# OpenVQE/OpenVQE

Measured on AMD Instinct MI355X. Metric: vqe_energy_evals_per_sec, higher is better.
Workload: dtype f64; 1 GPU; H2O/STO-3G UCCSD energy evaluation (the metric's config): 14 qubits, 140 generators = 1000 Pauli rotations, JW Hamiltonian 1086 terms / 162 x-groups; batch_per_gpu=65536, parallelism=batch-replicas x1

## Files before the change

openvqe_amd/backend.py:

```python
from __future__ import annotations

import ctypes
import os

import numpy as np

from . import _lib
from .operators import pack_string, pack_terms

GATE_OPCODES = {"X": 0, "H": 1, "RX": 2, "RY": 3, "RZ": 4, "CNOT": 5}
GRAD_FERMIONIC, GRAD_QUBIT = 0, 1
_REAL_TOL = 1e-12


def _real_coeff(c, what):
    c = complex(c)
    if abs(c.imag) > _REAL_TOL * max(1.0, abs(c.real)):
        raise ValueError(f"{what}: Pauli coefficient {c} is not real (generator must be Hermitian — "
                         "multiply the anti-Hermitian cluster operator by 1j, ref:openvqe/algorithms/ucc.py:30-31)")
    return c.real


def compile_ucc_program(nbqbits, generators, n_params=None):
    K = len(generators) if n_params is None else min(len(generators), int(n_params))
# ... 550 lines not shown
        cap = max(int(getattr(self, "_ham_terms", 0)), 1)
        got = np.full(cap, -1, np.int32)
        xb = np.zeros(cap, np.uint64)
        yb = np.zeros(cap, np.uint64)
        self._ck(self._L.ovqe_measure_groups(self._h, cap, got, xb, yb, ctypes.byref(G)))
        return got[:int(getattr(self, "_ham_terms", 0))], xb[:G.value], yb[:G.value]

    def energy_sampled(self, theta, n_shots, seed=0):
        K = self._K
        theta = np.ascontiguousarray(theta, np.float64).reshape(-1)[:K]
        if theta.shape[0] != K:
            raise ValueError(f"expected {K} parameters")
        e, s = ctypes.c_double(), ctypes.c_double()
        self._ck(self._L.ovqe_energy_sampled(self._h, theta if K else None, K, int(n_shots), int(seed), ctypes.byref(e), ctypes.byref(s)))
        return e.value, s.value

    def measure_info(self):
        out = (ctypes.c_int64 * 9)()
        self._ck(self._L.ovqe_measure_info(self._h, out, 9))
        keys = ("groups", "shots", "scratch_bytes", "launches", "basis_us", "scan_us", "draw_us", "terms", "high_passes")
        return dict(zip(keys, [int(v) for v in out]))

    def program_info(self):
        out = (ctypes.c_int64 * 38)()
        self._ck(self._L.ovqe_program_info(self._h, out, 38))
        keys = ("ops", "rotations", "literal_gates", "sweeps", "tiled_sweeps", "fused_ops", "support",
                "h_tile_sweeps", "h_untiled_groups", "h_entries", "h_merged_terms", "h_pair_terms_per_tile",
                "real_stream", "sp_ops", "sp_pairs", "sp_h_entries",
                "sector_support", "sector_sweeps", "sector_pairs", "sector_h_sweeps", "sector_h_elements", "sector_bytes",
                "sector_circuit_us", "sector_expect_us", "sector_h_stream_bytes", "sector_fci_block",
                "sp_conflicts_discovery_order", "sp_conflicts", "sector_regular_slot_bits", "sector_free_bits",
                "sp_h_pieces", "sp_h_slots", "sp_h_reads_per_state",
                "sp_lds_row_reads", "sp_lds_row_writes", "sp_lds_h_reads",
                "sp_lds_row_reads_discovery_order", "sp_lds_row_writes_discovery_order")
        return dict(zip(keys, [int(v) for v in out]))

    def rotation_program(self):
        n = ctypes.c_int64()
        self._ck(self._L.ovqe_get_rotation_program(self._h, 0, None, None, None, None, None, ctypes.byref(n)))
        R = n.value
        xs, zs = np.empty(R, np.uint64), np.empty(R, np.uint64)
        cs, p0, pi = np.empty(R, np.float64), np.empty(R, np.float64), np.empty(R, np.int32)
        self._ck(self._L.ovqe_get_rotation_program(self._h, R, xs.ctypes.data, zs.ctypes.data, cs.ctypes.data, p0.ctypes.data,
                                                   pi.ctypes.data, ctypes.byref(n)))
        return xs, zs, cs, p0, pi

    def pool_gradients(self, pool_ops, mode):
        cache = getattr(self, "_pool_cache", None)
        if cache is not None and cache[0] is pool_ops and cache[1] == len(pool_ops):
            offsets, xs, zs, cs = cache[2]
        else:
            offsets = np.zeros(len(pool_ops) + 1, np.int64)
            xs, zs, cs = [], [], []
            for k, op in enumerate(pool_ops):
                px, pz, pc = pack_terms(self.nbqbits, op.terms)
                xs.append(px)
                zs.append(pz)
# ... 34 lines not shown
```

openvqe_amd/csrc/ovqe_sv.hip:

```cpp
#include "../../include/ovqe_sv.h"

#include <hip/hip_runtime.h>

#include <algorithm>
#include <type_traits>
#include <atomic>
#include <cmath>
#include <cstdio>
#include <complex>
#include <cstring>
#include <map>
#include <memory>
#include <numeric>
#include <string>
#include <thread>
#include <chrono>
#include <vector>

#include "sv_kernels.hpp"
#include "sv_small.hpp"
#include "sv_sparse.hpp"
#include "sparse_pack.hpp"
#include "sv_tile.hpp"
#include "sv_sector.hpp"
// ... 259 lines not shown
    HamDev ham_adhoc;
    std::vector<uint64_t> adhoc_x, adhoc_z;
    std::vector<double> adhoc_c;
    bool prog_set = false;
    int32_t K = 0;
    uint64_t hf = 0;
    std::vector<SmallOp> ops;
    std::vector<SmallRot> rots;
    std::vector<SmallOp> sops;
    std::vector<SmallRot> srots;
    std::vector<int32_t> sop_src;
    std::vector<uint64_t> sop_zc;
    std::vector<SmallSeg> segs;
    DevBuf d_ops, d_rots, d_segs, d_stream;
    DevBuf d_rots_seq;
    std::vector<uint16_t> idx_stream;
    int cs_capacity = 512;
    DevBuf d_theta, d_energies, d_workspace;
    bool sp_tried = false, sp_valid = false;
    int sp_m = 0, sp_nops = 0, sp_nent = 0;
    int sp_nrows4 = 0;
    int sp_nprim = 0;
    DevBuf d_sp_rows, d_sp_rows64, d_sp_prim;
    int sp_nrows8 = 0;
    int sp_mp = 0, sp_hf = 0;
    int64_t sp_conflicts_before = 0, sp_conflicts_after = 0;
    int64_t sp_cycles[5] = {0, 0, 0, 0, 0};
    int64_t sp_npairs = 0;
    DevBuf d_sp_ops, d_sp_pairs, d_sp_entries;
    int sp_pack_inst = -1, sp_h_pieces = 0, sp_h_rpt = 0, sp_h_epr = 0;
    DevBuf d_sp_hpack;
    DevBuf d_pg_off, d_pg_xs, d_pg_terms, d_pg_out, d_pg_part;
    DevBuf d_pg_runs, d_pg_tabs;
    bool pg_tables = false;
    DevBuf d_nz_cnt, d_nz_start, d_nz_idx, d_nz_val, d_nz_bitmap;
    DevBuf d_exp_groups, d_exp_terms;
    std::vector<uint64_t> prev_x, prev_z;
    std::vector<double> prev_coeff, prev_phi0;
    std::vector<int32_t> prev_pidx;
    uint64_t prev_hf = 0;
    bool prog_extends_prev = false;
    uint32_t forms_used = 0;
    uint32_t sp_forms = 0;
    int64_t fused_launch[6] = {0, 0, 0, 0, 0, 0};
    bool nz_super = false, nz_super_prev = false, state_exposed = false;
    uint64_t nz_super_count = 0;
    DevBuf d_tile_smasks, d_tile_lists, d_tile_counts;
    int opt_screen_sparse = 16;
    int64_t last_exp_support = -1;
    int64_t last_screen_sector = 0;
    int64_t last_screen_support = -1;
    std::vector<int64_t> pg_off;
    std::vector<uint64_t> pg_xs;
    std::vector<HTerm> pg_terms;
    bool pg_valid = false;
    int opt_sparse = 1;
    int opt_sparse_spw = 0;
    int opt_sparse_pack = 1;
    int opt_sparse_dbg = 0;
    int opt_clifford_phase_host = 1;
    int opt_sparse_renumber = 1;
    int opt_sparse_rows = 1;
    int opt_sparse_wg = 1;
    int opt_sparse_shared = 1;
    int opt_sparse_grad = 1;
    DevBuf d_egroups, d_eterms, d_echunks, d_eflat;
    int exp_lbits = -1, exp_real = -1, exp_ngroups = 0, exp_nchunks = 0, exp_nflat = 0;
    int exp_ham_version = -1;
    hipEvent_t ev0 = nullptr, ev1 = nullptr;
    hipStream_t stream2 = nullptr;
    hipEvent_t ev_fork = nullptr, ev_join = nullptr;
    int opt_real_state = 0;
    CompactCover cc;
    int opt_compact = 1;
    int prog_version = 0;
    SectorEngine sec;
    SectorEngine scr;
    int scr_failed_version = -1;
    bool probe_independent = false;
    int opt_sector = 1;
    int opt_sector_bits = 0;
// ... 732 lines not shown
    return create_common(n_qubits, 0, 0, device, out);
} OVQE_CATCH(nullptr)

int ovqe_create_shard(int n_local, int n_global, uint64_t shard_index, int device, ovqe_handle *out) try {
    return create_common(n_local, n_global, shard_index, device, out);
} OVQE_CATCH(nullptr)

int ovqe_create_view(int n_qubits, int device, void *dev_ptr, ovqe_handle *out) try {
    if (!dev_ptr) return fail(nullptr, OVQE_ERR_INVALID, "dev_ptr is NULL");
    return create_common(n_qubits, 0, 0, device, out, dev_ptr);
} OVQE_CATCH(nullptr)

int ovqe_destroy(ovqe_handle h) try {
    OVQE_ENTER(h);
    if (!h) return OVQE_OK;
    (void)hipSetDevice(h->device);
    (void)hipStreamSynchronize(h->stream);
    if (h->own_state && h->state) (void)hipFree(h->state);
    for (int k = 0; k < 2; ++k)
        if (h->scratch[k]) (void)hipFree(h->scratch[k]);
    std::vector<DevBuf *> bufs = {&h->d_tile_cnt, &h->d_partials, &h->d_result, &h->d_rp, &h->d_ops, &h->d_rots, &h->d_rots_seq, &h->d_segs,
                                  &h->d_stream,
                                  &h->d_theta, &h->d_energies, &h->d_workspace, &h->d_egroups, &h->d_eterms, &h->d_echunks,
                                  &h->d_eflat, &h->d_sp_ops, &h->d_sp_rows, &h->d_sp_rows64, &h->d_sp_prim, &h->d_sp_pairs, &h->d_sp_entries, &h->d_sp_hpack, &h->d_pg_off, &h->d_pg_xs, &h->d_pg_terms, &h->d_pg_runs, &h->d_pg_tabs,
                                  &h->d_pg_out, &h->d_pg_part, &h->d_nz_cnt, &h->d_nz_start, &h->d_nz_idx, &h->d_nz_val, &h->d_nz_bitmap, &h->d_exp_groups, &h->d_exp_terms, &h->d_tile_smasks, &h->d_tile_lists, &h->d_tile_counts, &h->cc.d_sup, &h->cc.d_psic, &h->cc.d_loc, &h->cc.d_cid, &h->cc.d_off, &h->cc.d_sweeps};
    for (TilePlan *tp : {&h->tp, &h->tp_adhoc, &h->tp_real, &h->tp_adjoint}) bufs.insert(bufs.end(), {&tp->d_tops, &tp->d_trots});
    for (HamDev *H : {&h->ham, &h->ham_adhoc, &h->ham_real, &h->ham_conj})
        bufs.insert(bufs.end(), {&H->d_groups, &H->d_terms, &H->d_tchunks, &H->d_tgroups, &H->d_tterms, &H->d_tflats,
                                 &H->d_titems, &H->d_rest, &H->d_achunks, &H->d_agroups, &H->d_aterms, &H->d_dzin, &H->d_doff, &H->d_dterms});
    for (DevBuf *b : bufs)
        if (b->p) (void)hipFree(b->p);
    free_sector(h->sec);
    free_sector(h->scr);
    for (CrossSum *X : h->xsums) free_cross_sum(X);
    for (PoolPlan *P : h->xpools) free_pool_plan(P);
    free_rdm(h->rdm);
    free_metric(h->metric);
    free_measure(h->measure);
    free_subspace(h->subspace);
    h->kept_blocks.flush();
    if (h->h_rp) (void)hipHostFree(h->h_rp);
    if (h->h_result) (void)hipHostFree(h->h_result);
    if (h->h_io) (void)hipHostFree(h->h_io);
    if (h->h_fin) (void)hipHostFree(h->h_fin);
    if (h->ev0) (void)hipEventDestroy(h->ev0);
    if (h->ev1) (void)hipEventDestroy(h->ev1);
    if (h->ev_fork) (void)hipEventDestroy(h->ev_fork);
// ... 22 lines not shown
    OVQE_ENTER(h);
    if (!h || !name) return OVQE_ERR_INVALID;
    const std::string k(name);
    if (k == "force_path") h->opt_force_path = (int)value;
    else if (k == "real_state") h->opt_real_state = value ? 1 : 0;
    else if (k == "small_max_qubits") h->opt_small_max = (int)value;
    else if (k == "small_batch_max_qubits") h->opt_small_batch_max = (int)value;
    else if (k == "real_mode") {
        h->opt_real_mode = (int)value;
        h->sp_tried = false;
    }
    else if (k == "sparse") {
        h->opt_sparse = (int)value;
        h->sp_tried = false;
    }
    else if (k == "sparse_grad") h->opt_sparse_grad = value ? 1 : 0;
    else if (k == "sparse_renumber") {
        h->opt_sparse_renumber = value ? 1 : 0;
        h->sp_tried = false;
    }
#ifdef OVQE_TESTING
    else if (k == "sparse_spw") h->opt_sparse_spw = (int)value;
    else if (k == "sparse_dbg") h->opt_sparse_dbg = (int)value;
    else if (k == "sparse_pack") {
        h->opt_sparse_pack = value ? 1 : 0;
        h->sp_tried = false;
    }
#endif
    else if (k == "clifford_phase_host") h->opt_clifford_phase_host = (int)value;
    else if (k == "index_streams") {
        h->opt_index_streams = (int)value;
        if (h->prog_set) return finish_program(h);
    }
    else if (k == "sector" || k == "sector_bits" || k == "sector_max_gb" || k == "sector_min_qubits" || k == "sector_h" ||
             k == "sector_h_bits" || k == "sector_dict") {
        (k == "sector" ? h->opt_sector : k == "sector_bits" ? h->opt_sector_bits : k == "sector_max_gb" ? h->opt_sector_max_gb
         : k == "sector_h" ? h->opt_sector_h : k == "sector_h_bits" ? h->opt_sector_h_bits : k == "sector_dict" ? h->opt_sector_dict
                                                                                                              : h->opt_sector_min_qubits) = (int)value;
        reset_sector(h);
    }
    else if (k == "sector_threads") h->opt_sector_threads = (value == 0 || value == 64 || value == 512 || value == 1024) ? (int)value : 256;
#ifdef OVQE_TESTING
    else if (k == "sector_h_dbg") h->opt_sector_h_dbg = (int)value;
#endif
    else if (k == "sector_adjoint") h->opt_sector_adjoint = value == 1 ? 1 : (value == 2 ? 2 : 3);
    else if (k == "sector_batch") h->opt_sector_batch = (int)value;
// ... 256 lines not shown
    const TilePlan &TP = (real_on && h->tp_real_built) ? h->tp_real : h->tp;
    int64_t v[16] = {(int64_t)h->ops.size(), (int64_t)h->rots.size(), 0, (int64_t)TP.plan.size(),
                     (int64_t)TP.tsegs.size(), (int64_t)h->sops.size(),
                     !h->sp_tried ? -1 : (h->sp_valid ? (int64_t)h->sp_m : 0),
                     (int64_t)HI.tsweeps.size(), (int64_t)HI.n_rest, HI.tile_entries, HI.tile_terms, HI.tile_work,
                     real_on ? 1 : 0, h->sp_valid ? (int64_t)h->sp_nops : 0, h->sp_valid ? (int64_t)h->sp_npairs : 0,
                     h->sp_valid ? (int64_t)h->sp_nent : 0};
    for (const SmallOp &op : h->ops) v[2] += (op.kind == OP_X || op.kind == OP_H || op.kind == OP_CNOT);
    for (int i = 0; i < count && i < 16; ++i) info[i] = v[i];
    const SectorEngine &E = h->sec;
    const int64_t sv[14] = {E.valid ? (int64_t)E.K : 0, E.valid ? (int64_t)E.segs.size() : 0, E.valid ? (int64_t)E.npairs : 0,
                           E.valid ? (int64_t)E.hs.size() : 0, E.valid ? (int64_t)E.nnz : 0, E.valid ? (int64_t)E.bytes : 0,
                           E.valid ? (int64_t)(1e3 * E.last_circuit_ms) : 0, E.valid ? (int64_t)(1e3 * E.last_expect_ms) : 0,
                           E.valid ? (int64_t)E.h_stream_bytes : 0, E.valid ? (int64_t)E.last_fci_block : 0,
                            h->sp_valid ? h->sp_conflicts_before : 0, h->sp_valid ? h->sp_conflicts_after : 0,
                            (E.valid && E.regular && h->opt_sector_regular) ? (int64_t)E.reg_m : 0,
                            (E.valid && E.regular) ? (int64_t)__builtin_popcount(E.freemask) : 0};
    for (int i = 16; i < count && i < 30; ++i) info[i] = sv[i - 16];
    const bool packed = h->sp_valid && h->sp_pack_inst >= 0;
    const int64_t pv[3] = {packed ? (int64_t)h->sp_h_pieces : 0, packed ? (int64_t)h->sp_h_rpt * h->sp_h_epr : 0,
                           packed ? (int64_t)h->sp_h_rpt * (h->sp_h_epr + 1) : 0};
    for (int i = 30; i < count && i < 33; ++i) info[i] = pv[i - 30];
    for (int i = 33; i < count && i < 38; ++i) info[i] = h->sp_valid ? h->sp_cycles[i - 33] : 0;
    return OVQE_OK;
} OVQE_CATCH(h)

int ovqe_get_rotation_program(ovqe_handle h, int64_t capacity, uint64_t *x, uint64_t *z, double *coeff, double *phi0,
                              int32_t *pidx, int64_t *count) try {
    OVQE_ENTER(h);
    if (!h || !count || capacity < 0 || (capacity > 0 && (!x || !z || !coeff || !phi0 || !pidx))) return OVQE_ERR_INVALID;
    if (!h->prog_set) return fail(h, OVQE_ERR_STATE, "no program set");
    if (h->frame_open) return fail(h, OVQE_ERR_STATE, "the program's Clifford frame is open: the rotations alone are not the circuit");
    int64_t n = 0;
    for (const SmallOp &op : h->ops) {
        if (op.kind != OP_PAIR && op.kind != OP_DIAG) return fail(h, OVQE_ERR_STATE, "the program holds literal X / H / CNOT ops");
        for (int32_t r = op.first; r < op.first + op.count; ++r, ++n) {
            if (n >= capacity) continue;
            const SmallRot &sr = h->rots[r];
            x[n] = op.x;
            z[n] = sr.z;
            coeff[n] = sr.coeff;
            phi0[n] = sr.phi0;
            pidx[n] = sr.pidx;
        }
    }
    *count = n;
// ... 24 lines not shown
```

openvqe_amd/csrc/sparse_host.inc:

```

struct SharedInstance { int nw, ept, sstride, rpt, epr, te; };
constexpr SharedInstance SHARED_13 = {4, 13, 2568, 1, 17, 3};
constexpr SharedInstance SHARED_37 = {4, 37, 4104, 4, 10, 5};
constexpr SharedInstance SHARED_INSTANCES[2] = {SHARED_13, SHARED_37};

int build_sparse_program(ovqe_handle h) {
    h->sp_tried = true;
    h->sp_valid = false;
    if (!h->opt_sparse || !h->opt_table_fusion || !h->opt_real_mode || h->n_global != 0 || h->n_local > 40) return OVQE_OK;
    if (!h->prog_set || !h->ham.set || h->K <= 0) return OVQE_OK;
    for (const SmallRot &sr : h->rots)
        if (!(sr.ny & 1)) return OVQE_OK;
    for (const SmallOp &op : h->sops)
        if (op.kind != OP_TAB || op.count > 127) return OVQE_OK;
    const int MAXM = 4096;
    std::unordered_map<uint64_t, int> id;
    std::vector<uint64_t> S;
    auto get = [&](uint64_t a) {
        auto it = id.find(a);
        if (it != id.end()) return it->second;
        const int k = (int)S.size();
        id.emplace(a, k);
        S.push_back(a);
        return k;
// ... 49 lines not shown
            if (d == 0.0) continue;
            SpEntry e;
            e.ij = (uint32_t)k | ((uint32_t)kb << 12);
            e.pad = 0;
            e.c = x ? 2.0 * d : d;
            entries.push_back(e);
            if (entries.size() > (size_t)16 << 20) return OVQE_OK;
        }
    }
    SparsePlan plan;
    {
        std::vector<PlanOp> pops;
        for (const SpOp &so : ops) pops.push_back({so.first, so.npairs});
        plan_sparse_program(m, pops, pairs, h->opt_sparse_renumber != 0, &plan);
    }
    pairs.swap(plan.pairs);
    const int mp = plan.mp, hf_slot = plan.slot[0];
    h->sp_conflicts_before = plan.conflicts_discovery;
    h->sp_conflicts_after = plan.conflicts;
    for (SpEntry &e : entries) e.ij = (uint32_t)plan.slot[e.ij & 0xfffu] | ((uint32_t)plan.slot[(e.ij >> 12) & 0xfffu] << 12);
    arrange_entries(entries);
    std::vector<uint64_t> rows;
    h->sp_nrows4 = 0;
    const int ntab_all = (int)h->srots.size();
    std::vector<SmallRot> prim;
    std::vector<int> prim_of((size_t)ntab_all, -1);
    std::vector<uint8_t> prim_neg((size_t)ntab_all, 0);
    {
        std::unordered_map<uint64_t, std::vector<int>> by_param;
        for (int e = 0; e < ntab_all; ++e) {
            const SmallRot &sr = h->srots[e];
            std::vector<int> &cand = by_param[(uint64_t)(uint32_t)sr.pidx];
            for (int p : cand)
                if (std::fabs(prim[p].coeff) == std::fabs(sr.coeff) && prim[p].phi0 == 0.0 && sr.phi0 == 0.0) {
                    prim_of[e] = p;
                    prim_neg[e] = (prim[p].coeff < 0) != (sr.coeff < 0);
                    break;
                }
            if (prim_of[e] < 0) {
                prim_of[e] = (int)prim.size();
                cand.push_back((int)prim.size());
                prim.push_back(sr);
            }
        }
    }
    const int nprim = (int)prim.size();
// ... 3 lines not shown
            return (uint64_t)((uint32_t)(mp + lane) * 8u) | ((uint64_t)((uint32_t)(mp + 32 + lane) * 8u) << 16) |
                   ((uint64_t)((uint32_t)nprim * 16u) << 32);
        };
        size_t at = 0;
        for (const SpOp &so : ops)
            for (int c0 = 0; c0 < so.npairs; c0 += 32)
                for (int lane = 0; lane < 32; ++lane) {
                    const RowLane &rl = plan.rows[at++];
                    const uint64_t slots = (uint64_t)(rl.si * 8u) | ((uint64_t)(rl.sj * 8u) << 16);
                    if (rl.pair < 0) {
                        rows.push_back(slots | ((uint64_t)((uint32_t)nprim * 16u) << 32));
                        continue;
                    }
                    const uint32_t pw = pairs[(size_t)rl.pair], ent = (uint32_t)so.tab0 + (pw >> 25);
                    const bool neg = ((pw >> 24) & 1u) != (uint32_t)prim_neg[ent];
                    rows.push_back(slots | ((uint64_t)((uint32_t)prim_of[ent] * 16u) << 32) | (neg ? (1ull << 63) : 0ull));
                }
        const int nrows = (int)(rows.size() / 32);
        const int nrows4 = (nrows + 3) & ~3;
        for (int r = nrows; r < nrows4 + 4; ++r)
            for (int lane = 0; lane < 32; ++lane) rows.push_back(pad_word(lane));
        h->sp_nrows4 = nrows4;
        h->sp_nprim = nprim;
    }
    std::vector<uint64_t> rows64;
    h->sp_nrows8 = 0;
    if (h->opt_sparse_rows && (size_t)(mp + 128) * 8 < 65536 && (size_t)(nprim + 1) * 16 < 65536) {
        auto pad_word = [&](int lane) {
            return (uint64_t)((uint32_t)(mp + lane) * 8u) | ((uint64_t)((uint32_t)(mp + 64 + lane) * 8u) << 16) |
                   ((uint64_t)((uint32_t)nprim * 16u) << 32);
        };
        size_t at = 0;
        for (const SpOp &so : ops) {
            const int nch = (so.npairs + 31) / 32;
            for (int c = 0; c < nch; c += 2) {
                const int halves = std::min(2, nch - c);
                uint32_t ent0 = (uint32_t)nprim;
                for (int l = 0; l < 32 * halves; ++l)
                    if (plan.rows[at + l].pair >= 0) {
                        ent0 = (uint32_t)prim_of[(uint32_t)so.tab0 + (pairs[(size_t)plan.rows[at + l].pair] >> 25)];
                        break;
                    }
                for (int hh = 0; hh < 2; ++hh)
                    for (int l = 0; l < 32; ++l) {
                        if (hh >= halves) {
                            rows64.push_back((pad_word(32 + l) & 0xffffffffull) | ((uint64_t)(ent0 * 16u) << 32));
// ... 34 lines not shown
            ei[e] = entries[e].ij & 0xfffu;
            ej[e] = (entries[e].ij >> 12) & 0xfffu;
            ec[e] = entries[e].c;
        }
        const size_t state_bytes = (size_t)((mp + 64 + 1) & ~1) * sizeof(double);
        for (int k = 0; k < 2 && h->sp_pack_inst < 0; ++k) {
            const SharedInstance &I = SHARED_INSTANCES[k];
            const int nt = 64 * I.nw;
            if (entries.size() > (size_t)nt * I.ept || state_bytes > (size_t)I.sstride) continue;
            OwnerPack P;
            if (!pack_owner_pieces(ei, ej, ec, mp, nt, I.rpt, I.epr, &P)) continue;
            hpack.resize(P.c.size() * sizeof(double) + (P.oj.size() + P.oi.size()) * sizeof(uint16_t));
            std::memcpy(hpack.data(), P.c.data(), P.c.size() * sizeof(double));
            std::memcpy(hpack.data() + P.c.size() * sizeof(double), P.oj.data(), P.oj.size() * sizeof(uint16_t));
            std::memcpy(hpack.data() + P.c.size() * sizeof(double) + P.oj.size() * sizeof(uint16_t), P.oi.data(), P.oi.size() * sizeof(uint16_t));
            h->sp_pack_inst = k;
            h->sp_h_pieces = P.pieces;
            h->sp_h_rpt = I.rpt;
            h->sp_h_epr = I.epr;
            const PackCycles pc = pack_cycles(P);
            h->sp_cycles[2] = pc.slot_reads + pc.owner_reads;
        }
    }
    int rc = upload(h, h->d_sp_ops, ops.data(), ops.size() * sizeof(SpOp));
    if (!rc && h->sp_pack_inst >= 0) rc = upload(h, h->d_sp_hpack, hpack.data(), hpack.size());
    if (!rc && h->sp_nrows4) rc = upload(h, h->d_sp_rows, rows.data(), rows.size() * sizeof(uint64_t));
    if (!rc && (h->sp_nrows4 || h->sp_nrows8)) rc = upload(h, h->d_sp_prim, prim.data(), prim.size() * sizeof(SmallRot));
    if (!rc && h->sp_nrows8) rc = upload(h, h->d_sp_rows64, rows64.data(), rows64.size() * sizeof(uint64_t));
    if (!rc) rc = upload(h, h->d_sp_pairs, pairs.data(), pairs.size() * sizeof(uint32_t));
    if (!rc) rc = upload(h, h->d_sp_entries, entries.data(), entries.size() * sizeof(SpEntry));
    if (rc) return rc;
    h->sp_m = m;
    h->sp_mp = mp;
    h->sp_hf = hf_slot;
    h->sp_nops = (int)ops.size();
    h->sp_nent = (int)entries.size();
    h->sp_npairs = (int64_t)pairs.size();
    h->sp_valid = true;
    return OVQE_OK;
}

template <int SPW, bool STAGE = false>
int launch_sparse(ovqe_handle h, const SparseArgs &A, int grid, size_t smem) {
    if (int rc = lds_opt_in<&k_sparse_vqe<SPW, STAGE>>(h, LDS_WG_MAX)) return rc;
    hipLaunchKernelGGL((k_sparse_vqe<SPW, STAGE>), dim3(grid), dim3(64), smem, h->stream, A, h->cur_theta,
                       (const SmallRot *)h->d_rots.p, (const SpOp *)h->d_sp_ops.p, (const uint32_t *)h->d_sp_pairs.p,
                       (const SpEntry *)h->d_sp_entries.p, h->cur_energies);
    HIPC(h, hipGetLastError());
    return OVQE_OK;
}

enum : uint32_t {
    SPF_WG = 1u << 0,
    SPF_STAGED1 = 1u << 1,
    SPF_PLAIN1 = 1u << 2,
    SPF_ROWS2 = 1u << 3,
    SPF_PLAIN2 = 1u << 4,
    SPF_PLAIN4 = 1u << 5,
    SPF_GRAD_WG = 1u << 6,
    SPF_GRAD_STAGED = 1u << 7,
    SPF_GRAD_PLAIN = 1u << 8,
    SPF_DECLINED = 1u << 9,
    SPG_PER_WAVE = 1u << 10,
    SPG_SHARED_37 = 1u << 11,
    SPG_SHARED_13 = 1u << 12,
};

constexpr int64_t SHARED_MIN_B = 2048;

template <int NW, int RPT, int EPR, int SSTRIDE, int TE, int DBG>
int launch_rows_shared_dbg(ovqe_handle h, const SparseArgs &R, size_t smem) {
    constexpr int NS = 2 * NW;
    static std::atomic<uint32_t> per_dev[64];
    constexpr auto kern = &k_sparse_vqe_rows_shared<NW, RPT, EPR, SSTRIDE, TE, DBG>;
    constexpr size_t slots = (size_t)RPT * EPR * NW * 64;
    const double *hc = (const double *)h->d_sp_hpack.p;
    const uint16_t *ho = (const uint16_t *)(hc + slots);
    if (int rc = lds_opt_in<kern>(h, LDS_WG_MAX)) return rc;
    uint32_t pd = per_dev[h->device & 63].load(std::memory_order_relaxed);
    if ((pd >> 8) != smem) {
        int n = 0;
        HIPC(h, hipOccupancyMaxActiveBlocksPerMultiprocessor(&n, kern, NW * 64, smem));
        pd = (uint32_t)smem << 8 | (uint32_t)std::min(std::max(n, 1), 32 / NW);
        per_dev[h->device & 63].store(pd, std::memory_order_relaxed);
    }
    const int per_cu = (int)(pd & 255u);
    if (h->num_cus <= 0) {
        int cus = 0;
        if (hipDeviceGetAttribute(&cus, hipDeviceAttributeMultiprocessorCount, h->device) != hipSuccess || cus <= 0) cus = 256;
        h->num_cus = cus;
    }
    const int grid = (int)std::min<int64_t>((R.B + NS - 1) / NS, (int64_t)h->num_cus * per_cu);
    hipLaunchKernelGGL(kern, dim3(grid), dim3(NW * 64), smem, h->stream, R, h->cur_theta, (const SmallRot *)h->d_sp_prim.p,
                       (const uint64_t *)h->d_sp_rows.p, h->sp_nrows4, hc, ho, h->cur_energies);
    HIPC(h, hipGetLastError());
    return OVQE_OK;
}

template <int K>
int launch_rows_shared(ovqe_handle h, const SparseArgs &R, bool *taken) {
    constexpr SharedInstance I = SHARED_INSTANCES[K];
    constexpr int NW = I.nw, RPT = I.rpt, EPR = I.epr, SSTRIDE = I.sstride, TE = I.te;
    const size_t smem = sp_rows_shared_lds<NW, SSTRIDE>(R.ntab).bytes;
    *taken = h->sp_pack_inst == K && R.nent >= 1 && R.nent <= NW * 64 * I.ept && (size_t)R.mpad * sizeof(double) <= (size_t)SSTRIDE &&
             smem <= LDS_TWO_PER_CU;
    if (!*taken) return OVQE_OK;
#ifdef OVQE_TESTING
    switch (h->opt_sparse_dbg) {
    case 1: return launch_rows_shared_dbg<NW, RPT, EPR, SSTRIDE, TE, 1>(h, R, smem);
    case 2: return launch_rows_shared_dbg<NW, RPT, EPR, SSTRIDE, TE, 2>(h, R, smem);
    case 3: return launch_rows_shared_dbg<NW, RPT, EPR, SSTRIDE, TE, 3>(h, R, smem);
    case 4: return launch_rows_shared_dbg<NW, RPT, EPR, SSTRIDE, TE, 4>(h, R, smem);
    case 5: return launch_rows_shared_dbg<NW, RPT, EPR, SSTRIDE, TE, 5>(h, R, smem);
    default: break;
    }
#endif
    return launch_rows_shared_dbg<NW, RPT, EPR, SSTRIDE, TE, 0>(h, R, smem);
}

// ... 218 lines not shown
```

openvqe_amd/csrc/sparse_plan.hpp:

```cpp
#pragma once
#include <algorithm>
#include <cmath>
#include <cstdint>
#include <vector>

namespace ovqe {

inline int lds_access_cycles(const uint32_t *slot, int nlanes, int group, int banks) {
    int cycles = 0;
    for (int g0 = 0; g0 < nlanes; g0 += group) {
        const int gn = std::min(group, nlanes - g0);
        uint32_t s[64];
        int cnt[64] = {};
        std::copy(slot + g0, slot + g0 + gn, s);
        std::sort(s, s + gn);
        const int nu = (int)(std::unique(s, s + gn) - s);
        int worst = 0;
        for (int k = 0; k < nu; ++k) worst = std::max(worst, ++cnt[s[k] % (uint32_t)banks]);
        cycles += worst;
    }
    return cycles;
}
inline int lds_read_cycles(const uint32_t *slot32) { return lds_access_cycles(slot32, 32, 32, 32); }
inline int lds_write_cycles(const uint32_t *slot32) { return lds_access_cycles(slot32, 32, 16, 16); }
// ... 380 lines not shown
    for (int k = 0; k < m; ++k) P->slot[k] = k;
    P->mp = m;
    P->pairs = pairs;
    P->swapped.assign(pairs.size(), 0);
    plain_rows(ops, pairs, m, &P->rows);
    P->cycles = P->cycles_discovery = rows_cycles(P->rows);
    P->conflicts = P->conflicts_discovery = 0;
    if (!renumber || m <= 32 || m > 4064 || ops.empty()) return;
    P->conflicts_discovery = colliding_lane_pairs(ops, pairs, nullptr);
    plan_numbering(m, ops, pairs, &P->slot, &P->mp);
    std::vector<uint32_t> on_slots(pairs);
    for (uint32_t &pw : on_slots)
        pw = (pw & ~0xffffffu) | (uint32_t)P->slot[pair_i(pw)] | ((uint32_t)P->slot[pair_j(pw)] << 12);
    plan_rows(ops, on_slots, P->mp, &P->rows, &P->pairs, &P->swapped);
    P->cycles = rows_cycles(P->rows);
    P->conflicts = colliding_lane_pairs(ops, P->pairs, &P->swapped);
    for (size_t k = 0; k < P->pairs.size(); ++k)
        if (P->swapped[k]) {
            const uint32_t pw = P->pairs[k];
            P->pairs[k] = ((pw & ~0x1ffffffu) | pair_j(pw) | (pair_i(pw) << 12) | (pw & (1u << 24))) ^ (1u << 24);
        }
}

template <class E>
inline void arrange_entries(std::vector<E> &entries) {
    if (entries.size() <= 64) return;
    std::vector<std::vector<uint32_t>> by_bank(32);
    for (uint32_t e = 0; e < (uint32_t)entries.size(); ++e) by_bank[entries[e].ij & 31u].push_back(e);
    std::vector<E> arranged;
    arranged.reserve(entries.size());
    size_t left = entries.size();
    std::vector<uint32_t> order(32);
    while (left) {
        for (uint32_t b = 0; b < 32; ++b) order[b] = b;
        std::stable_sort(order.begin(), order.end(), [&](uint32_t a, uint32_t b) { return by_bank[a].size() > by_bank[b].size(); });
        uint32_t used_j = 0;
        size_t taken = 0;
        for (uint32_t bi : order) {
            std::vector<uint32_t> &lst = by_bank[bi];
            if (lst.empty()) continue;
            size_t pick = lst.size();
            for (size_t k = lst.size(); k-- > 0;) {
                const uint32_t bj = (entries[lst[k]].ij >> 12) & 31u;
                if (!((used_j >> bj) & 1u)) {
                    pick = k;
                    break;
// ... 36 lines not shown
```

openvqe_amd/csrc/sv_sparse.hpp:

```cpp
#pragma once
#include "sv_small.hpp"
#include "sv_metric_host.hpp"
#include "sv_wave_reduce.hpp"

namespace ovqe {

struct SpOp {
    int32_t first;
    int32_t npairs;
    int32_t tab0;
    int32_t pad;
};

struct SpEntry {
    uint32_t ij;
    uint32_t pad;
    double c;
};

struct SparseArgs {
    int m;
    int mpad;
    int K;
    int nops;
    int ntab;
    int nent;
// ... 184 lines not shown
            const SpEntry en = entries[e];
            const uint32_t ci = en.ij & 0xfffu, cj = (en.ij >> 12) & 0xfffu;
#pragma unroll
            for (int q = 0; q < SPW; ++q) acc[q] += en.c * st[(size_t)q * A.mpad + ci] * st[(size_t)q * A.mpad + cj];
        }
#pragma unroll
        for (int q = 0; q < SPW; ++q) {
            const double tot = DBG == 5 ? wave_sum(acc[q]) : wave_sum_lane0(WaveLanes{lane}, acc[q]);
            if (lane == 0 && b0 + q < A.B) energies[b0 + q] = tot + A.constant;
        }
        asm volatile("s_waitcnt lgkmcnt(0)" ::: "memory");
    }
}

struct SpRowsSharedLds { size_t cs, red, bytes; };
template <int NW, int SSTRIDE>
__host__ __device__ constexpr SpRowsSharedLds sp_rows_shared_lds(int ntab) {
    constexpr size_t NS = 2 * NW;
    const size_t cs = NS * SSTRIDE;
    const size_t red = cs + NS * (size_t)(ntab + 1) * sizeof(double2);
    return {cs, red, red + (size_t)NW * NS * sizeof(double)};
}

template <int NW, int RPT, int EPR, int SSTRIDE, int TE, int DBG = 0>
__global__ __launch_bounds__(NW * 64) void k_sparse_vqe_rows_shared(SparseArgs A, const double *__restrict__ theta,
                                                                    const SmallRot *__restrict__ tabrots, const uint64_t *__restrict__ rows,
                                                                    int nrows4, const double *__restrict__ hc, const uint16_t *__restrict__ ho,
                                                                    double *__restrict__ energies) {
    constexpr int NT = NW * 64, NS = 2 * NW, SD = SSTRIDE / 8;
    constexpr int TR = TE, TRN = TR ? TR : 1;
    static_assert(SSTRIDE % 8 == 0 && SSTRIDE % 512 != 0 && NS * SSTRIDE <= 65536 && (NS * SSTRIDE) % 16 == 0,
                  "state offsets are DS instruction immediates; a stride the ds_read2 forms cannot encode (see above)");
    static_assert(TE >= 0, "table records per lane");
    static_assert(NS == 8, "the transposed wave sums (wave_sums8) are built for eight states per workgroup");
    extern __shared__ __attribute__((aligned(16))) unsigned char smem[];
    const int ntab1 = A.ntab + 1;
    const SpRowsSharedLds L = sp_rows_shared_lds<NW, SSTRIDE>(A.ntab);
    double2 *cs = reinterpret_cast<double2 *>(smem + L.cs);
    double *red = reinterpret_cast<double *>(smem + L.red);
    const int tid = threadIdx.x, lane = tid & 63, wave = tid >> 6;
    const int s = lane >> 5, l = lane & 31, my = 2 * wave + s;
    unsigned char *sbase = smem + (size_t)my * SSTRIDE;
    double *sst = reinterpret_cast<double *>(sbase);
    double2 *csm = cs + (size_t)my * ntab1;
    unsigned char *cbase = reinterpret_cast<unsigned char *>(csm);
    constexpr int OPP = (EPR + 1) / 2;
    uint32_t oi[RPT], ojj[RPT][OPP];
    double ec[RPT][EPR];
#pragma unroll
    for (int r = 0; r < RPT; ++r) {
        oi[r] = ho[(size_t)(RPT * EPR + r) * NT + tid];
#pragma unroll
        for (int k = 0; k < EPR; ++k) ec[r][k] = hc[(size_t)(r * EPR + k) * NT + tid];
#pragma unroll
        for (int k = 0; k < OPP; ++k) {
            const uint32_t lo = ho[(size_t)(r * EPR + 2 * k) * NT + tid];
            const uint32_t hi = 2 * k + 1 < EPR ? ho[(size_t)(r * EPR + 2 * k + 1) * NT + tid] : 0u;
            ojj[r][k] = lo | (hi << 16);
        }
    }
    int32_t tp[TRN];
    double tc[TRN];
#pragma unroll
    for (int k = 0; k < TR; ++k) {
        const int e = l + 32 * k;
        const SmallRot sr = tabrots[e < A.ntab ? e : A.ntab - 1];
        tp[k] = sr.pidx;
        tc[k] = sr.coeff;
    }
    const int64_t nwork = (A.B + NS - 1) / NS;
    const uint64_t *rp = rows + l;
    auto theta_row = [&](int64_t w) {
        const int64_t b = w * NS + my;
        return theta + (b < A.B ? b : A.B - 1) * A.K;
    };
    auto fetch = [&](int64_t w, double (&tv)[TRN]) {
        const double *th = theta_row(w);
#pragma unroll
        for (int k = 0; k < TR; ++k) tv[k] = DBG == 4 ? 0.05 : th[tp[k]];
    };
    auto entry = [&](int e, double x) {
        double sn, c;
        if (DBG == 1) {
            sn = x;
            c = 1.0;
        } else {
            sincos(x, &sn, &c);
        }
        csm[e] = make_double2(c, sn);
    };
    auto table = [&](int64_t w, const double (&tv)[TRN]) {
#pragma unroll
        for (int k = 0; k < TR; ++k)
            if (l + 32 * k < A.ntab) entry(l + 32 * k, tc[k] * tv[k]);
        if (32 * TR < A.ntab) {
            const double *th = theta_row(w);
            for (int e = l + 32 * TR; e < A.ntab; e += 32) {
                const SmallRot sr = tabrots[e];
                entry(e, sr.coeff * (DBG == 4 ? 0.05 : th[sr.pidx]));
            }
        }
    };
    auto zero_fill = [&]() {
        for (int i = l; i < SD; i += 32) sst[i] = i == A.hf ? 1.0 : 0.0;
    };
    auto reduce = [&](int64_t b0) {
        if (tid < NS && b0 + tid < A.B) {
            double e = 0.0;
#pragma unroll
            for (int v = 0; v < NW; ++v) e += red[v * NS + tid];
            energies[b0 + tid] = e + A.constant;
        }
    };
    int64_t w = blockIdx.x, bprev = 0;
    if (w >= nwork) return;
    uint64_t w0 = rp[0], w1 = rp[32], w2 = rp[64], w3 = rp[96];
    double tv[TRN];
    fetch(w, tv);
    if (l == 0) csm[A.ntab] = make_double2(1.0, 0.0);
    zero_fill();
    for (bool first = true;; first = false) {
        table(w, tv);
        if (!first) {
            __syncthreads();
            reduce(bprev);
            zero_fill();
        }
        asm volatile("s_waitcnt lgkmcnt(0)" ::: "memory");
        auto cs_of = [&](uint64_t word) { return *reinterpret_cast<const double2 *>(cbase + ((uint32_t)(word >> 32) & 0xffffu)); };
        double2 tn = cs_of(w0);
        auto apply = [&](uint64_t word, uint64_t next) {
            const uint32_t lo = (uint32_t)word, hi = (uint32_t)(word >> 32);
            double *pi = reinterpret_cast<double *>(sbase + (lo & 0xffffu));
            double *pj = reinterpret_cast<double *>(sbase + (lo >> 16));
            const double2 t = tn;
            const double sn = __hiloint2double(__double2hiint(t.y) ^ (int)(hi & 0x80000000u), __double2loint(t.y));
            const double u = *pi, v = *pj;
            tn = cs_of(next);
            *pi = t.x * u + sn * v;
            *pj = t.x * v - sn * u;
            asm volatile("" ::: "memory");
        };
        auto trip = [&](const uint64_t *nx) {
            apply(w0, w1);
            w0 = nx[0];
            apply(w1, w2);
            w1 = nx[32];
            apply(w2, w3);
            w2 = nx[64];
            apply(w3, w0);
            w3 = nx[96];
        };
        if (DBG != 2) {
            for (int r = 0; r < nrows4 - 4; r += 4) trip(rp + (size_t)(r + 4) * 32);
            trip(rp);
        }
        const int64_t wnext = w + gridDim.x;
        const bool more = wnext < nwork;
        if (more) fetch(wnext, tv);
        __syncthreads();
        double acc[NS];
#pragma unroll
        for (int q = 0; q < NS; ++q) acc[q] = 0.0;
        if (DBG != 3) {
            constexpr int GPP = EPR + 1, G = RPT * GPP;
            auto goff = [&](int g) -> uint32_t {
// ... 483 lines not shown
```

Measured before the change: 185.7 million evals/s.

## Fuse adjacent sparse rotation ops into three-slot chain rows in LDS

Adds a host planner that merges each pair of consecutive sparse rotation ops whose pairs form disjoint chains into a single row of three-slot lanes, cutting the number of LDS round trips. A new CHAIN variant of the shared-memory kernel reads 12-byte row words and applies two chained Givens rotations per lane, with bank-conflict-aware lane placement and spare slots for padding. This is enabled by default. In exchange the row stream is wider, each lane does more LDS accesses, and a wave-uniform branch decides per row whether it is fused.

```diff
diff --git a/openvqe_amd/backend.py b/openvqe_amd/backend.py
--- a/openvqe_amd/backend.py
+++ b/openvqe_amd/backend.py
@@ -596,8 +596,8 @@
         return dict(zip(keys, [int(v) for v in out]))
 
     def program_info(self):
-        out = (ctypes.c_int64 * 38)()
-        self._ck(self._L.ovqe_program_info(self._h, out, 38))
+        out = (ctypes.c_int64 * 40)()
+        self._ck(self._L.ovqe_program_info(self._h, out, 40))
         keys = ("ops", "rotations", "literal_gates", "sweeps", "tiled_sweeps", "fused_ops", "support",
                 "h_tile_sweeps", "h_untiled_groups", "h_entries", "h_merged_terms", "h_pair_terms_per_tile",
                 "real_stream", "sp_ops", "sp_pairs", "sp_h_entries",
@@ -606,7 +606,8 @@
                 "sp_conflicts_discovery_order", "sp_conflicts", "sector_regular_slot_bits", "sector_free_bits",
                 "sp_h_pieces", "sp_h_slots", "sp_h_reads_per_state",
                 "sp_lds_row_reads", "sp_lds_row_writes", "sp_lds_h_reads",
-                "sp_lds_row_reads_discovery_order", "sp_lds_row_writes_discovery_order")
+                "sp_lds_row_reads_discovery_order", "sp_lds_row_writes_discovery_order",
+                "sp_round_trips", "sp_chain_rows")
         return dict(zip(keys, [int(v) for v in out]))
 
     def rotation_program(self):
diff --git a/openvqe_amd/csrc/ovqe_sv.hip b/openvqe_amd/csrc/ovqe_sv.hip
--- a/openvqe_amd/csrc/ovqe_sv.hip
+++ b/openvqe_amd/csrc/ovqe_sv.hip
@@ -305,6 +305,8 @@
     int sp_nrows4 = 0;
     int sp_nprim = 0;
     DevBuf d_sp_rows, d_sp_rows64, d_sp_prim;
+    DevBuf d_sp_crows;
+    int sp_crows4 = 0, sp_round_trips = 0, sp_chain_rows = 0;
     int sp_nrows8 = 0;
     int sp_mp = 0, sp_hf = 0;
     int64_t sp_conflicts_before = 0, sp_conflicts_after = 0;
@@ -340,6 +342,7 @@
     int opt_sparse = 1;
     int opt_sparse_spw = 0;
     int opt_sparse_pack = 1;
+    int opt_sparse_fuse = 1;
     int opt_sparse_dbg = 0;
     int opt_clifford_phase_host = 1;
     int opt_sparse_renumber = 1;
@@ -1118,7 +1121,7 @@
     std::vector<DevBuf *> bufs = {&h->d_tile_cnt, &h->d_partials, &h->d_result, &h->d_rp, &h->d_ops, &h->d_rots, &h->d_rots_seq, &h->d_segs,
                                   &h->d_stream,
                                   &h->d_theta, &h->d_energies, &h->d_workspace, &h->d_egroups, &h->d_eterms, &h->d_echunks,
-                                  &h->d_eflat, &h->d_sp_ops, &h->d_sp_rows, &h->d_sp_rows64, &h->d_sp_prim, &h->d_sp_pairs, &h->d_sp_entries, &h->d_sp_hpack, &h->d_pg_off, &h->d_pg_xs, &h->d_pg_terms, &h->d_pg_runs, &h->d_pg_tabs,
+                                  &h->d_eflat, &h->d_sp_ops, &h->d_sp_rows, &h->d_sp_crows, &h->d_sp_rows64, &h->d_sp_prim, &h->d_sp_pairs, &h->d_sp_entries, &h->d_sp_hpack, &h->d_pg_off, &h->d_pg_xs, &h->d_pg_terms, &h->d_pg_runs, &h->d_pg_tabs,
                                   &h->d_pg_out, &h->d_pg_part, &h->d_nz_cnt, &h->d_nz_start, &h->d_nz_idx, &h->d_nz_val, &h->d_nz_bitmap, &h->d_exp_groups, &h->d_exp_terms, &h->d_tile_smasks, &h->d_tile_lists, &h->d_tile_counts, &h->cc.d_sup, &h->cc.d_psic, &h->cc.d_loc, &h->cc.d_cid, &h->cc.d_off, &h->cc.d_sweeps};
     for (TilePlan *tp : {&h->tp, &h->tp_adhoc, &h->tp_real, &h->tp_adjoint}) bufs.insert(bufs.end(), {&tp->d_tops, &tp->d_trots});
     for (HamDev *H : {&h->ham, &h->ham_adhoc, &h->ham_real, &h->ham_conj})
@@ -1187,6 +1190,7 @@
 #ifdef OVQE_TESTING
     else if (k == "sparse_spw") h->opt_sparse_spw = (int)value;
     else if (k == "sparse_dbg") h->opt_sparse_dbg = (int)value;
+    else if (k == "sparse_fuse") h->opt_sparse_fuse = value ? 1 : 0;
     else if (k == "sparse_pack") {
         h->opt_sparse_pack = value ? 1 : 0;
         h->sp_tried = false;
@@ -1489,6 +1493,8 @@
                            packed ? (int64_t)h->sp_h_rpt * (h->sp_h_epr + 1) : 0};
     for (int i = 30; i < count && i < 33; ++i) info[i] = pv[i - 30];
     for (int i = 33; i < count && i < 38; ++i) info[i] = h->sp_valid ? h->sp_cycles[i - 33] : 0;
+    if (count > 38) info[38] = h->sp_valid ? h->sp_round_trips : 0;
+    if (count > 39) info[39] = h->sp_valid ? h->sp_chain_rows : 0;
     return OVQE_OK;
 } OVQE_CATCH(h)
 
diff --git a/openvqe_amd/csrc/sparse_host.inc b/openvqe_amd/csrc/sparse_host.inc
--- a/openvqe_amd/csrc/sparse_host.inc
+++ b/openvqe_amd/csrc/sparse_host.inc
@@ -95,6 +95,7 @@
     arrange_entries(entries);
     std::vector<uint64_t> rows;
     h->sp_nrows4 = 0;
+    h->sp_crows4 = h->sp_round_trips = h->sp_chain_rows = 0;
     const int ntab_all = (int)h->srots.size();
     std::vector<SmallRot> prim;
     std::vector<int> prim_of((size_t)ntab_all, -1);
@@ -144,6 +145,7 @@
             for (int lane = 0; lane < 32; ++lane) rows.push_back(pad_word(lane));
         h->sp_nrows4 = nrows4;
         h->sp_nprim = nprim;
+        h->sp_round_trips = nrows;
     }
     std::vector<uint64_t> rows64;
     h->sp_nrows8 = 0;
@@ -224,7 +226,43 @@
             h->sp_cycles[2] = pc.slot_reads + pc.owner_reads;
         }
     }
+    std::vector<uint32_t> crows;
+    if (h->sp_pack_inst >= 0) {
+        std::vector<PlanOp> pops;
+        std::vector<int32_t> tab0_of((size_t)pairs.size(), 0);
+        for (const SpOp &so : ops) {
+            pops.push_back({so.first, so.npairs});
+            for (int k = 0; k < so.npairs; ++k) tab0_of[(size_t)so.first + k] = so.tab0;
+        }
+        plan.pairs = pairs;
+        ChainTable T;
+        plan_chain_rows(pops, plan, &T);
+        if (T.nfused > 0) {
+            const uint32_t ident = (uint32_t)nprim * 16u;
+            auto entry = [&](int32_t pair, uint32_t flip) -> uint32_t {
+                if (pair < 0) return ident | flip;
+                const uint32_t pw = pairs[(size_t)pair], ent = (uint32_t)tab0_of[(size_t)pair] + (pw >> 25);
+                return (uint32_t)prim_of[ent] * 16u | ((((pw >> 24) & 1u) ^ flip ^ (uint32_t)prim_neg[ent]) & 1u);
+            };
+            for (const ChainLane &cl : T.lanes) {
+                crows.push_back(cl.a * 8u | (cl.b * 8u) << 16);
+                crows.push_back(entry(cl.pa, cl.fa) | entry(cl.kind ? cl.pb : -1, cl.kind ? cl.fb : 0u) << 16);
+                crows.push_back(cl.kind ? (cl.c * 8u | 1u << 16) : 0u);
+            }
+            const int crows4 = (T.nrows + 3) & ~3;
+            for (int r = T.nrows; r < crows4 + 4; ++r)
+                for (int lane = 0; lane < 32; ++lane) {
+                    crows.push_back((uint32_t)(mp + lane) * 8u | ((uint32_t)(mp + 32 + lane) * 8u) << 16);
+                    crows.push_back(ident | ident << 16);
+                    crows.push_back(0u);
+                }
+            h->sp_crows4 = crows4;
+            h->sp_round_trips = T.nrows;
+            h->sp_chain_rows = T.nchain;
+        }
+    }
     int rc = upload(h, h->d_sp_ops, ops.data(), ops.size() * sizeof(SpOp));
+    if (!rc && h->sp_crows4) rc = upload(h, h->d_sp_crows, crows.data(), crows.size() * sizeof(uint32_t));
     if (!rc && h->sp_pack_inst >= 0) rc = upload(h, h->d_sp_hpack, hpack.data(), hpack.size());
     if (!rc && h->sp_nrows4) rc = upload(h, h->d_sp_rows, rows.data(), rows.size() * sizeof(uint64_t));
     if (!rc && (h->sp_nrows4 || h->sp_nrows8)) rc = upload(h, h->d_sp_prim, prim.data(), prim.size() * sizeof(SmallRot));
@@ -270,11 +308,11 @@
 
 constexpr int64_t SHARED_MIN_B = 2048;
 
-template <int NW, int RPT, int EPR, int SSTRIDE, int TE, int DBG>
-int launch_rows_shared_dbg(ovqe_handle h, const SparseArgs &R, size_t smem) {
+template <int NW, int RPT, int EPR, int SSTRIDE, int TE, int DBG, bool CHAIN>
+int launch_rows_shared_tab(ovqe_handle h, const SparseArgs &R, size_t smem) {
     constexpr int NS = 2 * NW;
     static std::atomic<uint32_t> per_dev[64];
-    constexpr auto kern = &k_sparse_vqe_rows_shared<NW, RPT, EPR, SSTRIDE, TE, DBG>;
+    constexpr auto kern = &k_sparse_vqe_rows_shared<NW, RPT, EPR, SSTRIDE, TE, DBG, CHAIN>;
     constexpr size_t slots = (size_t)RPT * EPR * NW * 64;
     const double *hc = (const double *)h->d_sp_hpack.p;
     const uint16_t *ho = (const uint16_t *)(hc + slots);
@@ -294,9 +332,15 @@
     }
     const int grid = (int)std::min<int64_t>((R.B + NS - 1) / NS, (int64_t)h->num_cus * per_cu);
     hipLaunchKernelGGL(kern, dim3(grid), dim3(NW * 64), smem, h->stream, R, h->cur_theta, (const SmallRot *)h->d_sp_prim.p,
-                       (const uint64_t *)h->d_sp_rows.p, h->sp_nrows4, hc, ho, h->cur_energies);
+                       (const uint64_t *)(CHAIN ? h->d_sp_crows.p : h->d_sp_rows.p), CHAIN ? h->sp_crows4 : h->sp_nrows4, hc, ho, h->cur_energies);
     HIPC(h, hipGetLastError());
     return OVQE_OK;
+}
+
+template <int NW, int RPT, int EPR, int SSTRIDE, int TE, int DBG>
+int launch_rows_shared_dbg(ovqe_handle h, const SparseArgs &R, size_t smem) {
+    if (h->sp_crows4 && h->opt_sparse_fuse) return launch_rows_shared_tab<NW, RPT, EPR, SSTRIDE, TE, DBG, true>(h, R, smem);
+    return launch_rows_shared_tab<NW, RPT, EPR, SSTRIDE, TE, DBG, false>(h, R, smem);
 }
 
 template <int K>
diff --git a/openvqe_amd/csrc/sparse_plan.hpp b/openvqe_amd/csrc/sparse_plan.hpp
--- a/openvqe_amd/csrc/sparse_plan.hpp
+++ b/openvqe_amd/csrc/sparse_plan.hpp
@@ -426,6 +426,253 @@
         }
 }
 
+struct ChainLane {
+    uint32_t a, b, c;
+    int32_t pa, pb;
+    uint32_t fa, fb;
+    uint32_t kind;
+};
+
+struct ChainTable {
+    std::vector<ChainLane> lanes;
+    std::vector<uint8_t> fused;
+    int nrows = 0, nchain = 0, nfused = 0;
+    RowCycles cycles;
+};
+
+inline void plan_chain_rows(const std::vector<PlanOp> &ops, const SparsePlan &P, ChainTable *T) {
+    const int nh = (int)ops.size();
+    const uint32_t NONE = 0xffffffffu;
+    T->lanes.clear();
+    T->fused.assign((size_t)nh, 0);
+    T->nrows = T->nchain = T->nfused = 0;
+    T->cycles = RowCycles();
+    std::vector<size_t> row0((size_t)nh + 1, 0);
+    for (int o = 0; o < nh; ++o) row0[(size_t)o + 1] = row0[o] + (size_t)((ops[o].npairs + 31) / 32);
+    std::vector<int32_t> owner((size_t)P.mp + 64, -1);
+    struct Comp { uint32_t a, b, c; int32_t pa, pb; uint32_t fa, fb; };
+    auto account = [&](const ChainLane *row) {
+        uint32_t s[3][32];
+        for (int l = 0; l < 32; ++l) {
+            s[0][l] = row[l].a;
+            s[1][l] = row[l].b;
+            s[2][l] = row[l].c;
+        }
+        for (int k = 0; k < (row[0].kind ? 3 : 2); ++k) {
+            T->cycles.reads += lds_read_cycles(s[k]);
+            T->cycles.writes += lds_write_cycles(s[k]);
+        }
+    };
+    for (int o = 0; o < nh;) {
+        std::vector<Comp> comp;
+        bool fuse = o + 1 < nh;
+        if (fuse) {
+            const PlanOp &A = ops[o], &B = ops[(size_t)o + 1];
+            for (int k = 0; k < A.npairs; ++k) {
+                const uint32_t pw = P.pairs[(size_t)A.first + k];
+                owner[pair_i(pw)] = owner[pair_j(pw)] = k;
+                comp.push_back({pair_i(pw), pair_j(pw), NONE, A.first + k, -1, 0u, 1u});
+            }
+            for (int k = 0; k < B.npairs && fuse; ++k) {
+                const uint32_t pw = P.pairs[(size_t)B.first + k], i = pair_i(pw), j = pair_j(pw);
+                const int32_t ci = owner[i], cj = owner[j];
+                if (ci >= 0 && cj >= 0) {
+                    fuse = false;
+                } else if (ci < 0 && cj < 0) {
+                    comp.push_back({NONE, i, j, -1, B.first + k, 0u, 0u});
+                } else {
+                    Comp &c = comp[(size_t)(ci >= 0 ? ci : cj)];
+                    const uint32_t shared = ci >= 0 ? i : j;
+                    if (c.pb >= 0) {
+                        fuse = false;
+                        break;
+                    }
+                    if (c.a == shared) {
+                        std::swap(c.a, c.b);
+                        c.fa = 1u;
+                    }
+                    c.c = ci >= 0 ? j : i;
+                    c.pb = B.first + k;
+                    c.fb = ci >= 0 ? 0u : 1u;
+                }
+            }
+            for (int k = 0; k < A.npairs; ++k) {
+                const uint32_t pw = P.pairs[(size_t)A.first + k];
+                owner[pair_i(pw)] = owner[pair_j(pw)] = -1;
+            }
+            fuse = fuse && ((int)comp.size() + 31) / 32 < (A.npairs + 31) / 32 + (B.npairs + 31) / 32;
+        }
+        if (!fuse) {
+            for (size_t r = row0[o]; r < row0[(size_t)o + 1]; ++r) {
+                ChainLane row[32];
+                for (int l = 0; l < 32; ++l) {
+                    const RowLane &rl = P.rows[r * 32 + (size_t)l];
+                    row[l] = {rl.si, rl.sj, 0u, rl.pair, -1, 0u, 0u, 0u};
+                }
+                account(row);
+                T->lanes.insert(T->lanes.end(), row, row + 32);
+                ++T->nrows;
+            }
+            o += 1;
+            continue;
+        }
+        T->fused[o] = 1;
+        ++T->nfused;
+        const int nc = (int)comp.size(), nch = (nc + 31) / 32;
+        auto side = [](const Comp &c, int s) { return s == 0 ? c.a : s == 1 ? c.b : c.c; };
+        std::vector<std::vector<int>> chunk((size_t)nch);
+        {
+            std::vector<int> cnt((size_t)nch * 96, 0);
+            for (int t = 0; t < nc; ++t) {
+                int best = -1, best_over = 0;
+                for (int c = 0; c < nch; ++c) {
+                    if (chunk[c].size() >= 32) continue;
+                    int over = 0;
+                    for (int s = 0; s < 3; ++s)
+                        if (side(comp[t], s) != NONE) over += cnt[(size_t)c * 96 + (size_t)s * 32 + (side(comp[t], s) & 31u)];
+                    if (best < 0 || over < best_over || (over == best_over && chunk[c].size() < chunk[best].size())) {
+                        best = c;
+                        best_over = over;
+                    }
+                }
+                chunk[best].push_back(t);
+                for (int s = 0; s < 3; ++s)
+                    if (side(comp[t], s) != NONE) ++cnt[(size_t)best * 96 + (size_t)s * 32 + (side(comp[t], s) & 31u)];
+            }
+        }
+        for (int c = 0; c < nch; ++c) {
+            std::vector<int> half[2];
+            int cnt16[2][3][16] = {};
+            for (int t : chunk[c]) {
+                int over[2] = {0, 0};
+                for (int hs = 0; hs < 2; ++hs)
+                    for (int s = 0; s < 3; ++s)
+                        if (side(comp[t], s) != NONE) over[hs] += cnt16[hs][s][side(comp[t], s) & 15u];
+                int hs = over[1] < over[0] || (over[1] == over[0] && half[1].size() < half[0].size()) ? 1 : 0;
+                if (half[hs].size() >= 16) hs ^= 1;
+                half[hs].push_back(t);
+                for (int s = 0; s < 3; ++s)
+                    if (side(comp[t], s) != NONE) ++cnt16[hs][s][side(comp[t], s) & 15u];
+            }
+            {
+                auto cost = [&]() {
+                    int cycles = 0, beyond = 0;
+                    for (int hs = 0; hs < 2; ++hs)
+                        for (int s = 0; s < 3; ++s) {
+                            int worst = 0;
+                            for (int r = 0; r < 16; ++r) {
+                                worst = std::max(worst, cnt16[hs][s][r]);
+                                beyond += std::max(0, cnt16[hs][s][r] - 1);
+                            }
+                            cycles += worst;
+                        }
+                    return 1024 * cycles + beyond;
+                };
+                auto count = [&](int hs, int t, int d) {
+                    for (int s = 0; s < 3; ++s)
+                        if (side(comp[t], s) != NONE) cnt16[hs][s][side(comp[t], s) & 15u] += d;
+                };
+                int best = cost();
+                for (int pass = 0, moved = 1; moved && pass < 64; ++pass) {
+                    moved = 0;
+                    for (int hs = 0; hs < 2; ++hs)
+                        for (size_t q = 0; q < half[hs].size(); ++q) {
+                            const int t = half[hs][q];
+                            count(hs, t, -1);
+                            count(hs ^ 1, t, 1);
+                            if (half[hs ^ 1].size() < 16 && cost() < best) {
+                                best = cost();
+                                half[hs ^ 1].push_back(t);
+                                half[hs].erase(half[hs].begin() + (long)q);
+                                moved = 1;
+                                --q;
+                                continue;
+                            }
+                            bool done = false;
+                            for (size_t p = 0; p < half[hs ^ 1].size() && !done; ++p) {
+                                const int u = half[hs ^ 1][p];
+                                if (u == t) continue;
+                                count(hs ^ 1, u, -1);
+                                count(hs, u, 1);
+                                if (cost() < best) {
+                                    best = cost();
+                                    std::swap(half[hs][q], half[hs ^ 1][p]);
+                                    done = true;
+                                    moved = 1;
+                                } else {
+                                    count(hs ^ 1, u, 1);
+                                    count(hs, u, -1);
+                                }
+                            }
+                            if (!done) {
+                                count(hs, t, 1);
+                                count(hs ^ 1, t, -1);
+                            }
+                        }
+                }
+            }
+            ChainLane row[32];
+            bool filled[32] = {};
+            uint32_t used32[3] = {0, 0, 0}, used16[2][3] = {{0, 0, 0}, {0, 0, 0}};
+            for (int hs = 0; hs < 2; ++hs)
+                for (size_t q = 0; q < half[hs].size(); ++q) {
+                    const int l = 16 * hs + (int)q;
+                    const Comp &k = comp[(size_t)half[hs][q]];
+                    filled[l] = true;
+                    row[l] = {k.a, k.b, k.c, k.pa, k.pb, k.fa, k.fb, 1u};
+                    for (int s = 0; s < 3; ++s)
+                        if (side(k, s) != NONE) {
+                            used32[s] |= 1u << (side(k, s) & 31u);
+                            used16[hs][s] |= 1u << (side(k, s) & 15u);
+                        }
+                }
+            uint64_t spare_taken = 0;
+            auto spare = [&](int l, int s) {
+                int pick = -1, grade = -1;
+                for (int q = 0; q < 64; ++q) {
+                    if ((spare_taken >> q) & 1u) continue;
+                    const uint32_t sl = (uint32_t)P.mp + (uint32_t)q;
+                    const int g = 2 * !((used32[s] >> (sl & 31u)) & 1u) + !((used16[l >> 4][s] >> (sl & 15u)) & 1u);
+                    if (g > grade) {
+                        grade = g;
+                        pick = q;
+                    }
+                }
+                spare_taken |= 1ull << pick;
+                const uint32_t sl = (uint32_t)P.mp + (uint32_t)pick;
+                used32[s] |= 1u << (sl & 31u);
+                used16[l >> 4][s] |= 1u << (sl & 15u);
+                return sl;
+            };
+            for (int l = 0; l < 32; ++l) {
+                if (!filled[l]) {
+                    const uint32_t e = spare(l, 0), mid = spare(l, 1);
+                    row[l] = {e, mid, NONE, -1, -1, 0u, 1u, 1u};
+                } else if (row[l].a == NONE) {
+                    row[l].a = spare(l, 0);
+                } else if (row[l].c == NONE) {
+                    row[l].c = spare(l, 2);
+                }
+            }
+            for (int l = 0; l < 32; ++l)
+                if (row[l].c == NONE) {
+                    if (spare_taken != ~0ull) {
+                        row[l].c = spare(l, 2);
+                    } else {
+                        row[l].c = row[l].a;
+                        used32[2] |= 1u << (row[l].c & 31u);
+                        used16[l >> 4][2] |= 1u << (row[l].c & 15u);
+                    }
+                }
+            account(row);
+            T->lanes.insert(T->lanes.end(), row, row + 32);
+            ++T->nrows;
+            ++T->nchain;
+        }
+        o += 2;
+    }
+}
+
 template <class E>
 inline void arrange_entries(std::vector<E> &entries) {
     if (entries.size() <= 64) return;
diff --git a/openvqe_amd/csrc/sv_sparse.hpp b/openvqe_amd/csrc/sv_sparse.hpp
--- a/openvqe_amd/csrc/sv_sparse.hpp
+++ b/openvqe_amd/csrc/sv_sparse.hpp
@@ -2,6 +2,7 @@
 #include "sv_small.hpp"
 #include "sv_metric_host.hpp"
 #include "sv_wave_reduce.hpp"
+#include <type_traits>
 
 namespace ovqe {
 
@@ -232,7 +233,15 @@
     return {cs, red, red + (size_t)NW * NS * sizeof(double)};
 }
 
-template <int NW, int RPT, int EPR, int SSTRIDE, int TE, int DBG = 0>
+__device__ __forceinline__ void sp_rotate(double c, double sn, double u, double v, double &ru, double &rv) {
+    ru = fma(c, u, __dmul_rn(sn, v));
+    rv = fma(c, v, -__dmul_rn(sn, u));
+}
+__device__ __forceinline__ double sp_signed(double x, uint32_t sign31) {
+    return __hiloint2double(__double2hiint(x) ^ (int)(sign31 & 0x80000000u), __double2loint(x));
+}
+
+template <int NW, int RPT, int EPR, int SSTRIDE, int TE, int DBG = 0, bool CHAIN = false>
 __global__ __launch_bounds__(NW * 64) void k_sparse_vqe_rows_shared(SparseArgs A, const double *__restrict__ theta,
                                                                     const SmallRot *__restrict__ tabrots, const uint64_t *__restrict__ rows,
                                                                     int nrows4, const double *__restrict__ hc, const uint16_t *__restrict__ ho,
@@ -279,7 +288,8 @@
         tc[k] = sr.coeff;
     }
     const int64_t nwork = (A.B + NS - 1) / NS;
-    const uint64_t *rp = rows + l;
+    using RowWord = typename std::conditional<CHAIN, uint3, uint64_t>::type;
+    const RowWord *rp = reinterpret_cast<const RowWord *>(rows) + l;
     auto theta_row = [&](int64_t w) {
         const int64_t b = w * NS + my;
         return theta + (b < A.B ? b : A.B - 1) * A.K;
@@ -324,7 +334,7 @@
     };
     int64_t w = blockIdx.x, bprev = 0;
     if (w >= nwork) return;
-    uint64_t w0 = rp[0], w1 = rp[32], w2 = rp[64], w3 = rp[96];
+    RowWord w0 = rp[0], w1 = rp[32], w2 = rp[64], w3 = rp[96];
     double tv[TRN];
     fetch(w, tv);
     if (l == 0) csm[A.ntab] = make_double2(1.0, 0.0);
@@ -337,21 +347,54 @@
             zero_fill();
         }
         asm volatile("s_waitcnt lgkmcnt(0)" ::: "memory");
-        auto cs_of = [&](uint64_t word) { return *reinterpret_cast<const double2 *>(cbase + ((uint32_t)(word >> 32) & 0xffffu)); };
-        double2 tn = cs_of(w0);
-        auto apply = [&](uint64_t word, uint64_t next) {
-            const uint32_t lo = (uint32_t)word, hi = (uint32_t)(word >> 32);
+        auto cs_at = [&](uint32_t off) { return *reinterpret_cast<const double2 *>(cbase + off); };
+        auto cs_a = [&](const RowWord &word) {
+            if constexpr (CHAIN) return cs_at(word.y & 0xfff0u);
+            else return cs_at((uint32_t)(word >> 32) & 0xffffu);
+        };
+        double2 tn = cs_a(w0), tnb = tn;
+        if constexpr (CHAIN) tnb = cs_at((w0.y >> 16) & 0xfff0u);
+        auto apply = [&](const RowWord &word, const RowWord &next) {
+            uint32_t lo, sa;
+            if constexpr (CHAIN) {
+                lo = word.x;
+                sa = word.y << 31;
+            } else {
+                lo = (uint32_t)word;
+                sa = (uint32_t)(word >> 32);
+            }
             double *pi = reinterpret_cast<double *>(sbase + (lo & 0xffffu));
             double *pj = reinterpret_cast<double *>(sbase + (lo >> 16));
             const double2 t = tn;
-            const double sn = __hiloint2double(__double2hiint(t.y) ^ (int)(hi & 0x80000000u), __double2loint(t.y));
+            const double sn = sp_signed(t.y, sa);
+            if constexpr (CHAIN) {
+                if (__builtin_amdgcn_readfirstlane(word.z) >> 16) {
+                    double *pc = reinterpret_cast<double *>(sbase + (word.z & 0xffffu));
+                    const double2 tb = tnb;
+                    const double snb = sp_signed(tb.y, word.y << 15);
+                    const double u = *pi, v = *pj, x = *pc;
+                    tn = cs_a(next);
+                    tnb = cs_at((next.y >> 16) & 0xfff0u);
+                    double ru, rv, rw, rx;
+                    sp_rotate(t.x, sn, u, v, ru, rv);
+                    sp_rotate(tb.x, snb, rv, x, rw, rx);
+                    *pi = ru;
+                    *pj = rw;
+                    *pc = rx;
+                    asm volatile("" ::: "memory");
+                    return;
+                }
+            }
             const double u = *pi, v = *pj;
-            tn = cs_of(next);
-            *pi = t.x * u + sn * v;
-            *pj = t.x * v - sn * u;
+            tn = cs_a(next);
+            if constexpr (CHAIN) tnb = cs_at((next.y >> 16) & 0xfff0u);
+            double ru, rv;
+            sp_rotate(t.x, sn, u, v, ru, rv);
+            *pi = ru;
+            *pj = rv;
             asm volatile("" ::: "memory");
         };
-        auto trip = [&](const uint64_t *nx) {
+        auto trip = [&](const RowWord *nx) {
             apply(w0, w1);
             w0 = nx[0];
             apply(w1, w2);
```

Result: no change. 187.1 million evals/s (median of 6 runs) (+0.7%).
